# Sagnac/OpticalRayTracing.jl

Measured on NVIDIA B200. Metric: FP64 ray-surface intersections/sec, higher is better.
Workload: dtype f64

## Files before the change

opticalraytracing.jl_b200/csrc/kern_trace3d.cu:

```cuda
#include "kern.cuh"

struct Hit {
    double xs, ys;
    double xf, yf;
    unsigned flags;
    double opl;
};

__device__ __forceinline__ double strict_opl_start(const RayS& r, int mode, double n0, double y, double x, double z0)
{
    if (mode == 1) return SD(SM(n0, -z0), r.k3);
    return SM(n0, SA(SM(x, r.k1), SM(y, r.k2)));
}

__device__ __forceinline__ double strict_opl_close(const RayS& r, const ort_field& f, double nlast)
{
    if (f.opd_radius == 0.0) return r.opl;
    const double qx = SS(r.x, f.opd_xc), qy = SS(r.y, f.opd_yc);
    const double b = SA(SM(qx, r.k1), SM(qy, r.k2));
    const double cq = SS(SA(SM(qx, qx), SM(qy, qy)), SM(f.opd_radius, f.opd_radius));
    const double sg = (f.opd_radius < 0.0) ? -1.0 : 1.0;
    const double tau = SS(-b, SM(sg, SQ(SS(SM(b, b), cq))));
    return SA(r.opl, SM(nlast, tau));
}
// ... 45 lines not shown
    const Hit h = trace_strict_impl<EXT, SurfArray, POLY, true>(S, nsurf, stop, y, x, u, v, fld, n0, nlast, vignette, poly, npoly, &bad);
    if (bad) return trace_strict_cold<EXT, SurfArray, POLY>(S, nsurf, stop, y, x, u, v, fld, n0, nlast, vignette, poly, npoly);
    return h;
}

__device__ __forceinline__ int nonfinite_bit(double a) { return 0x7FEFFFFF - (hi32(a) & 0x7FFFFFFF); }

__device__ __forceinline__ bool is_nan_bits(double a)
{
    return (hi32(a) & 0x7FFFFFFF) > 0x7FF00000 ||
           ((hi32(a) & 0x7FFFFFFF) == 0x7FF00000 && __double2loint(a) != 0);
}

template <int RPT, bool EXT, class SurfArray, bool MIRROR = true, int SIMPLE = 0, bool R2ONLY = false, int POLY = 0, class QT = NoPolyK>
__device__ __forceinline__ void trace_fast(const SurfArray& S, int nsurf, int stop, double n0,
                                           const double* y, const double* x, const double* u,
                                           const double* v, Hit* h, int* amb,
                                           const ort_field* fld = nullptr, double nlast = 1.0, bool vignette = false,
                                           const double* K0 = nullptr, bool kzcheck = true, const double* poly = nullptr,
                                           int npoly = 0, const QT* Q = nullptr)
{
    RaysF<RPT> r;
#pragma unroll
    for (int j = 0; j < RPT; j++) {
        if (K0) {
            r.x[j] = x[j]; r.y[j] = y[j]; r.z[j] = 0.0;
            r.Kx[j] = K0[0]; r.Ky[j] = K0[1]; r.Kz[j] = K0[2];
            r.amb[j] = 0; r.opl[j] = 0.0; r.vig[j] = 0;
        } else fast_init(r, j, n0, y[j], x[j], u[j], v[j]);
        if (EXT) {
            r.opl[j] = (fld->mode == 1) ? fast_div(-(n0 * n0) * fld->z0, r.Kz[j]) : fma(x[j], r.Kx[j], y[j] * r.Ky[j]);
        }
    }
    int i = 0;
    for (; i < stop; i++)
        if constexpr (POLY == 2) fast_step<RPT, EXT, MIRROR, SIMPLE, 2>(S[i], r, vignette, nullptr, 0, 0, &Q->r[i]);
        else fast_step<RPT, EXT, MIRROR, SIMPLE, POLY>(S[i], r, vignette, (POLY && poly) ? poly + (size_t)i * npoly : nullptr, npoly, nsurf * npoly);
#pragma unroll
    for (int j = 0; j < RPT; j++) {
        if (R2ONLY) { h[j].xs = fma(r.x[j], r.x[j], r.y[j] * r.y[j]); h[j].ys = 0.0; }
        else { h[j].xs = r.x[j]; h[j].ys = r.y[j]; }
    }
    for (; i < nsurf; i++)
        if constexpr (POLY == 2) fast_step<RPT, EXT, MIRROR, SIMPLE, 2>(S[i], r, vignette, nullptr, 0, 0, &Q->r[i]);
        else fast_step<RPT, EXT, MIRROR, SIMPLE, POLY>(S[i], r, vignette, (POLY && poly) ? poly + (size_t)i * npoly : nullptr, npoly, nsurf * npoly);
#pragma unroll
    for (int j = 0; j < RPT; j++) {
        h[j].xf = r.x[j]; h[j].yf = r.y[j];
        h[j].flags = (EXT && r.vig[j]) ? ORT_FLAG_VIGN : 0u;
        amb[j] = r.amb[j] | nonfinite_bit(r.x[j]) | nonfinite_bit(r.y[j]);
        if (kzcheck) amb[j] |= nonfinite_bit(r.Kz[j]);
        h[j].opl = 0.0;
        if (EXT) {
            double opl = r.opl[j];
            if (fld->opd_radius != 0.0) {
                const double qx = r.x[j] - fld->opd_xc, qy = r.y[j] - fld->opd_yc;
                const double bK = fma(qx, r.Kx[j], qy * r.Ky[j]);
                const double cq = fma(qx, qx, fma(qy, qy, -fld->opd_radius * fld->opd_radius));
                const double d = fma(bK, bK, -(nlast * nlast) * cq);
                double sq = fast_sqrt(d);
                if ((fld->opd_radius < 0.0) != (nlast < 0.0)) sq = -sq;
                opl = opl - bK - sq;
                amb[j] |= nonfinite_bit(opl);
            }
            h[j].opl = opl;
        }
    }
}

struct RawAcc {
    int n, nflag_lo, nflag_hi;
    double s1x, s2x, s1y, s2y, rmax;
    double s1o, s2o; int nvig;
    int nstrict;
// ... 490 lines not shown
    const unsigned nxu = (unsigned)A.nx;

    for (unsigned tile = blockIdx.x; tile < ntiles; tile += gridDim.x) {
        double y0[RPT], x0[RPT], u[RPT], v[RPT];
        unsigned idx[RPT];
        bool valid[RPT];
#pragma unroll
        for (int j = 0; j < RPT; j++) {
            const unsigned i0 = (tile * RPT + j) * ORT_TILE + threadIdx.x;
            valid[j] = i0 < NN;
            idx[j] = min(i0, NN - 1);
            const unsigned iy = idx[j] / nxu, ix = idx[j] - iy * nxu;
            y0[j] = __ldg(A.ys + (ysoff + iy)); x0[j] = __ldg(A.xs + ix);
            u[j] = 0.0; v[j] = 0.0;
        }
        if (!collimated || ARITH != ORT_ARITH_FAST) {
#pragma unroll
            for (int j = 0; j < RPT; j++) field_slopes(fld, y0[j], x0[j], u[j], v[j]);
        }
        FocusRay q[RPT];
        double xs[RPT], ys[RPT];
        unsigned flg[RPT];
        bool sv[RPT];
        if (ARITH == ORT_ARITH_FAST) {
            RaysF<RPT> r;
#pragma unroll
            for (int j = 0; j < RPT; j++) {
                if (collimated) {
                    r.x[j] = x0[j]; r.y[j] = y0[j]; r.z[j] = 0.0;
                    r.Kx[j] = K0[0]; r.Ky[j] = K0[1]; r.Kz[j] = K0[2];
                    r.amb[j] = 0; r.opl[j] = 0.0; r.vig[j] = 0;
                } else fast_init(r, j, P.n0, y0[j], x0[j], u[j], v[j]);
            }
            const int ns = P.nsurf - 1;
            int i = 0;
            for (; i < A.stop; i++) fast_step<RPT, false, MIRROR, SIMPLE, 0>(P.s[i], r);
#pragma unroll
            for (int j = 0; j < RPT; j++) s_xy[j][threadIdx.x] = make_double2(r.x[j], r.y[j]);
            for (; i < ns; i++) fast_step<RPT, false, MIRROR, SIMPLE, 0>(P.s[i], r);
#pragma unroll
            for (int j = 0; j < RPT; j++) {
                int amb = r.amb[j];
                if (refr_last) {
                    const double Dp = fma(r.Kz[j], r.Kz[j], SL.dn2);
                    amb |= hi32(Dp) - SL.tir_thr;
                    amb |= nonfinite_bit(MIRROR ? sign_of_n2(fast_sqrt(Dp), SL.n2mask) : fast_sqrt(Dp));
                }
                q[j].a0 = r.x[j]; q[j].a1 = r.y[j]; q[j].a2 = r.z[j]; q[j].a3 = r.Kx[j]; q[j].a4 = r.Ky[j];
                q[j].a5 = fast_div_rcp(r.Kz[j]);
                double xa, ya, xb, yb;
                focus_pos_fast(q[j], F.t_lo, xa, ya);
                focus_pos_fast(q[j], F.t_hi, xb, yb);
                amb |= nonfinite_bit(xa) | nonfinite_bit(ya) | nonfinite_bit(xb) | nonfinite_bit(yb);
                const double2 st = s_xy[j][threadIdx.x];
                const double r2 = fma(st.x, st.x, st.y * st.y);
                amb |= tiny_vs_bit(r2 - A.a_stop2, A.a_stop2);
                sv[j] = amb < 0;
                flg[j] = 0u;
            }
        } else {
#pragma unroll
            for (int j = 0; j < RPT; j++) {
                int bad = 0;
                FocusS o = focus_strict_impl<ORT_STRICT_XF>(P, A.stop, y0[j], x0[j], u[j], v[j], &bad);
                if (ORT_STRICT_XF && bad) o = focus_strict_cold(P, A.stop, y0[j], x0[j], u[j], v[j]);
                q[j] = o.q; xs[j] = o.xs; ys[j] = o.ys; flg[j] = o.flags; sv[j] = true;
// ... 435 lines not shown
        double s1x = 0.0, s2x = 0.0, s1y = 0.0, s2y = 0.0, rmax = -CUDART_INF;
        const unsigned edge_b = (unsigned)(A.ny - 1) * nxu;
        if (AIMED && ok && threadIdx.x < 2) {
            double ex, ey, rr; bool keep;
            if (rec[14] == 1.0) { const double* e = rec + 16 + 4 * threadIdx.x; keep = e[0] == 1.0; ex = e[1]; ey = e[2]; rr = e[3]; }
            else {
                const Hit he = trace_strict_cold<false>(s_surf, nsurf, stop, threadIdx.x ? par[1] : par[0], 0.0, par[7], A.v);
                const double ri = jl_hypot(he.xs, he.ys);
                keep = !(ri > par[5] || is_nan_bits(he.xf) || is_nan_bits(he.yf)); ex = he.xf; ey = he.yf - par[8]; rr = ri * ri;
            }
            if (keep) { const double dy = ey - cy; s1x += ex; s2x = fma(ex, ex, s2x); s1y += dy; s2y = fma(dy, dy, s2y); rmax = fmax(rmax, rr); n++; }
        }
        unsigned iyj[CS_RPT], ixj[CS_RPT];
#pragma unroll
        for (int j = 0; j < CS_RPT; j++) { const unsigned i = threadIdx.x + j * CS_THREADS; iyj[j] = i / nxu; ixj[j] = i - iyj[j] * nxu; }
        const double g_y1 = par[0], g_y2 = par[1], g_dy = par[2], g_xe = par[3], g_dx = par[4], a_stop2 = par[6], hpc = par[8] + cy;
        for (unsigned i0 = threadIdx.x; ok && i0 < NN; i0 += step) {
            double y0[CS_RPT], x0[CS_RPT], uu[CS_RPT], vv[CS_RPT];
            bool valid[CS_RPT];
#pragma unroll
            for (int j = 0; j < CS_RPT; j++) {
                const unsigned i = i0 + j * CS_THREADS;
                valid[j] = i < NN && !(AIMED && (i == 0 || i == edge_b));
                const unsigned iy = min(iyj[j], (unsigned)A.ny - 1), ix = ixj[j];
                if (AIMED) {
                    y0[j] = (iy == (unsigned)A.ny - 1) ? g_y2 : SA(g_y1, SM((double)iy, g_dy));
                    x0[j] = (ix == nxu - 1) ? g_xe : SM((double)ix, g_dx);
                } else { y0[j] = __ldg(A.ys + iy); x0[j] = __ldg(A.xs + ix); }
                uu[j] = 0.0; vv[j] = A.v;
                ixj[j] += dr; iyj[j] += dq;
                if (ixj[j] >= nxu) { ixj[j] -= nxu; iyj[j]++; }
            }
            Hit h[CS_RPT]; int amb[CS_RPT];
            trace_fast<CS_RPT, false, SurfK*, false, SIMPLE>(s_surf, nsurf, stop, n0, y0, x0, uu, vv, h, amb, nullptr, 1.0, false, K0);
#pragma unroll
            for (int j = 0; j < CS_RPT; j++) {
                double r2 = fma(h[j].xs, h[j].xs, h[j].ys * h[j].ys);
                amb[j] |= tiny_vs_bit(r2 - a_stop2, a_stop2);
                bool drop = r2 > a_stop2;
                if (amb[j] < 0 && valid[j]) {
                    h[j] = trace_strict_cold<false>(s_surf, nsurf, stop, y0[j], x0[j], par[7], A.v);
                    const double ri = jl_hypot(h[j].xs, h[j].ys);
                    drop = ri > par[5] || is_nan_bits(h[j].xf) || is_nan_bits(h[j].yf);
                    r2 = ri * ri;
                }
                if (valid[j] && !drop) {
                    const double ex = h[j].xf, dy = h[j].yf - hpc;
                    s1x += ex; s2x = fma(ex, ex, s2x); s1y += dy; s2y = fma(dy, dy, s2y);
                    if (r2 > rmax) rmax = r2;
                    n++;
                }
            }
        }
#pragma unroll
        for (int d = 16; d >= 1; d >>= 1) {
            n += __shfl_down_sync(0xffffffffu, n, d);
            s1x += __shfl_down_sync(0xffffffffu, s1x, d); s2x += __shfl_down_sync(0xffffffffu, s2x, d);
            s1y += __shfl_down_sync(0xffffffffu, s1y, d); s2y += __shfl_down_sync(0xffffffffu, s2y, d);
            rmax = fmax(rmax, __shfl_down_sync(0xffffffffu, rmax, d));
        }
        const int lane = threadIdx.x & 31, warp = threadIdx.x >> 5;
        if (lane == 0) { s_redn[warp] = n; s_red[warp][0] = s1x; s_red[warp][1] = s2x; s_red[warp][2] = s1y; s_red[warp][3] = s2y; s_red[warp][4] = rmax; }
        __syncthreads();
        if (threadIdx.x == 0) {
            for (int w = 1; w < CS_THREADS / 32; w++) {
                n += s_redn[w]; s1x += s_red[w][0]; s2x += s_red[w][1]; s1y += s_red[w][2]; s2y += s_red[w][3];
            }
// ... 58 lines not shown
    return arith == ORT_ARITH_FAST ? (variant == 2 ? ORT_SIMPLE_RPT : (variant == 3 ? ORT_SE_RPT : (variant == 4 ? ORT_SC_RPT : ORT_FAST_RPT))) : ORT_STRICT_RPT;
}

int grid_blocks_per_sm(int arith, int variant)
{
    int nb = 0;
    cudaError_t e;
    if (arith == ORT_ARITH_FAST && variant == 2)
        e = cudaOccupancyMaxActiveBlocksPerMultiprocessor(&nb, k_grid<ORT_ARITH_FAST, ORT_SIMPLE_RPT, 0, 1, false, true>, ORT_TILE, 0);
    else if (arith == ORT_ARITH_FAST && variant == 3)
        e = cudaOccupancyMaxActiveBlocksPerMultiprocessor(&nb, k_grid<ORT_ARITH_FAST, ORT_SE_RPT, 2, 0, false, true>, ORT_TILE, 0);
    else if (arith == ORT_ARITH_FAST && variant == 4)
        e = cudaOccupancyMaxActiveBlocksPerMultiprocessor(&nb, k_grid<ORT_ARITH_FAST, ORT_SC_RPT, 0, 1, false, 2>, ORT_TILE, 0);
    else if (arith == ORT_ARITH_FAST)
        e = variant ? cudaOccupancyMaxActiveBlocksPerMultiprocessor(&nb, k_grid<ORT_ARITH_FAST, ORT_FAST_RPT, 1>, ORT_TILE, 0)
                    : cudaOccupancyMaxActiveBlocksPerMultiprocessor(&nb, k_grid<ORT_ARITH_FAST, ORT_FAST_RPT, 0>, ORT_TILE, 0);
    else
        e = (variant & 1) ? cudaOccupancyMaxActiveBlocksPerMultiprocessor(&nb, k_grid<ORT_ARITH_STRICT, ORT_STRICT_RPT, 1>, ORT_TILE, 0)
                          : cudaOccupancyMaxActiveBlocksPerMultiprocessor(&nb, k_grid<ORT_ARITH_STRICT, ORT_STRICT_RPT, 0>, ORT_TILE, 0);
    if (e != cudaSuccess || nb < 1) nb = 1;
    return nb;
}

cudaError_t launch_grid(const Presc& P, const GridArgs& A, int arith, dim3 grid, cudaStream_t st, const PolyK* Q)
{
    const bool ext = A.ext != 0 || P.poly != nullptr;
    if (arith == ORT_ARITH_FAST) {
        const bool others = A.r || A.theta || A.wx || A.wy || A.flags || A.opd;
        const bool lean = !ext && !others && A.ex && A.ey && A.mask;
        const bool stats_only = !ext && !others && !A.ex && !A.ey && !A.mask;
        const int variant = grid_variant(P, arith, ext);
        const bool simple = variant == 2;
        const bool lean_opd = (A.ext & ORT_EXT_OPD) && A.ex && A.ey && A.mask && A.opd && !(A.r || A.theta || A.wx || A.wy || A.flags);
        if (variant == 3 && !(A.ext & ORT_EXT_VIGNETTE) && lean_opd) k_grid<ORT_ARITH_FAST, ORT_SE_RPT, 2, 1, false, true><<<grid, ORT_TILE, 0, st>>>(P, A, NoPolyK());
        else if (variant == 3 && !(A.ext & ORT_EXT_VIGNETTE)) k_grid<ORT_ARITH_FAST, ORT_SE_RPT, 2, 0, false, true><<<grid, ORT_TILE, 0, st>>>(P, A, NoPolyK());
        else if (variant == 3 && lean_opd) k_grid<ORT_ARITH_FAST, ORT_SE_RPT, 1, 1, false, true><<<grid, ORT_TILE, 0, st>>>(P, A, NoPolyK());
        else if (variant == 3) k_grid<ORT_ARITH_FAST, ORT_SE_RPT, 1, 0, false, true><<<grid, ORT_TILE, 0, st>>>(P, A, NoPolyK());
        else if (variant == 4 && lean) k_grid<ORT_ARITH_FAST, ORT_SC_RPT, 0, 1, false, 2><<<grid, ORT_TILE, 0, st>>>(P, A, NoPolyK());
        else if (variant == 4 && stats_only) k_grid<ORT_ARITH_FAST, ORT_SC_RPT, 0, 2, false, 2><<<grid, ORT_TILE, 0, st>>>(P, A, NoPolyK());
        else if (variant == 4) k_grid<ORT_ARITH_FAST, ORT_SC_RPT, 0, 0, false, 2><<<grid, ORT_TILE, 0, st>>>(P, A, NoPolyK());
        else if (simple && lean) k_grid<ORT_ARITH_FAST, ORT_SIMPLE_RPT, 0, 1, false, true><<<grid, ORT_TILE, 0, st>>>(P, A, NoPolyK());
        else if (simple && stats_only) k_grid<ORT_ARITH_FAST, ORT_SIMPLE_RPT, 0, 2, false, true><<<grid, ORT_TILE, 0, st>>>(P, A, NoPolyK());
        else if (simple) k_grid<ORT_ARITH_FAST, ORT_SIMPLE_RPT, 0, 0, false, true><<<grid, ORT_TILE, 0, st>>>(P, A, NoPolyK());
        else if (P.poly && Q && !A.ext && !others && A.ex && A.ey && A.mask) k_grid<ORT_ARITH_FAST, ORT_FAST_RPT, 0, 1, false, 0, 2><<<grid, ORT_TILE, 0, st>>>(P, A, *Q);
        else if (P.poly && Q) k_grid<ORT_ARITH_FAST, ORT_FAST_RPT, 1, 0, false, 0, 2><<<grid, ORT_TILE, 0, st>>>(P, A, *Q);
        else if (P.poly && !A.ext && !others && A.ex && A.ey && A.mask) k_grid<ORT_ARITH_FAST, ORT_FAST_RPT, 0, 1, false, 0, 1><<<grid, ORT_TILE, 0, st>>>(P, A, NoPolyK());
        else if (P.poly) k_grid<ORT_ARITH_FAST, ORT_FAST_RPT, 1, 0, false, 0, 1><<<grid, ORT_TILE, 0, st>>>(P, A, NoPolyK());
        else if (ext && !P.has_mirror) k_grid<ORT_ARITH_FAST, ORT_FAST_RPT, 1, 0, false><<<grid, ORT_TILE, 0, st>>>(P, A, NoPolyK());
        else if (ext) k_grid<ORT_ARITH_FAST, ORT_FAST_RPT, 1><<<grid, ORT_TILE, 0, st>>>(P, A, NoPolyK());
        else if (lean && !P.has_mirror) k_grid<ORT_ARITH_FAST, ORT_FAST_RPT, 0, 1, false><<<grid, ORT_TILE, 0, st>>>(P, A, NoPolyK());
        else if (stats_only && !P.has_mirror) k_grid<ORT_ARITH_FAST, ORT_FAST_RPT, 0, 2, false><<<grid, ORT_TILE, 0, st>>>(P, A, NoPolyK());
        else if (!P.has_mirror) k_grid<ORT_ARITH_FAST, ORT_FAST_RPT, 0, 0, false><<<grid, ORT_TILE, 0, st>>>(P, A, NoPolyK());
        else if (lean) k_grid<ORT_ARITH_FAST, ORT_FAST_RPT, 0, 1><<<grid, ORT_TILE, 0, st>>>(P, A, NoPolyK());
        else if (stats_only) k_grid<ORT_ARITH_FAST, ORT_FAST_RPT, 0, 2><<<grid, ORT_TILE, 0, st>>>(P, A, NoPolyK());
        else k_grid<ORT_ARITH_FAST, ORT_FAST_RPT, 0><<<grid, ORT_TILE, 0, st>>>(P, A, NoPolyK());
    } else {
        if (ext) k_grid<ORT_ARITH_STRICT, ORT_STRICT_RPT, 1><<<grid, ORT_TILE, 0, st>>>(P, A, NoPolyK());
        else k_grid<ORT_ARITH_STRICT, ORT_STRICT_RPT, 0><<<grid, ORT_TILE, 0, st>>>(P, A, NoPolyK());
    }
    return cudaGetLastError();
}

cudaError_t launch_grid_finalize(const RawPart* partials, int nparts, int n_fields, ort_stats* stats,
                                 cudaStream_t st)
{
    k_grid_finalize<<<n_fields, 256, 0, st>>>(partials, nparts, stats);
    return cudaGetLastError();
}

size_t compact_tile_ints(unsigned NN)
{
    const size_t ntiles = (NN + ORT_TILE - 1) / ORT_TILE;
    return ntiles + ntiles / SCAN_CHUNK + 2;
}

static cudaError_t launch_tile_scan(int* tile_counts, unsigned ntiles, int n_fields, cudaStream_t st)
{
    const unsigned nchunks = (ntiles + SCAN_CHUNK - 1) / SCAN_CHUNK;
    k_tile_scan<<<dim3(nchunks, n_fields), 256, 0, st>>>(tile_counts, tile_counts + (size_t)n_fields * ntiles, ntiles, nchunks);
    k_chunk_scan<<<n_fields, 256, 0, st>>>(tile_counts + (size_t)n_fields * ntiles, nchunks);
    return cudaGetLastError();
}

cudaError_t launch_compact(int* tile_counts, const CompactArgs& C, int n_fields, cudaStream_t st)
{
    const unsigned ntiles = (C.NN + ORT_TILE - 1) / ORT_TILE;
    cudaError_t e = launch_tile_scan(tile_counts, ntiles, n_fields, st);
    if (e != cudaSuccess) return e;
    k_compact<<<dim3(ntiles, n_fields), ORT_TILE, 0, st>>>(C);
    return cudaGetLastError();
}

int focus_blocks_per_sm(int arith, int variant)
{
    int nb = 0;
    cudaError_t e;
    if (arith != ORT_ARITH_FAST) e = cudaOccupancyMaxActiveBlocksPerMultiprocessor(&nb, k_focus<ORT_ARITH_STRICT, ORT_STRICT_RPT, true, 0>, ORT_TILE, 0);
    else if (variant == 2) e = cudaOccupancyMaxActiveBlocksPerMultiprocessor(&nb, k_focus<ORT_ARITH_FAST, ORT_SIMPLE_RPT, false, 1>, ORT_TILE, 0);
    else if (variant == 4) e = cudaOccupancyMaxActiveBlocksPerMultiprocessor(&nb, k_focus<ORT_ARITH_FAST, ORT_SC_RPT, false, 2>, ORT_TILE, 0);
    else e = cudaOccupancyMaxActiveBlocksPerMultiprocessor(&nb, k_focus<ORT_ARITH_FAST, ORT_FAST_RPT, true, 0>, ORT_TILE, 0);
    if (e != cudaSuccess || nb < 1) nb = 1;
    return nb;
}

cudaError_t launch_focus(const Presc& P, const FocusArgs& F, int arith, dim3 grid, cudaStream_t st)
{
    if (arith == ORT_ARITH_FAST) {
        const int variant = grid_variant(P, arith, 0);
        if (variant == 2) k_focus<ORT_ARITH_FAST, ORT_SIMPLE_RPT, false, 1><<<grid, ORT_TILE, 0, st>>>(P, F);
        else if (variant == 4) k_focus<ORT_ARITH_FAST, ORT_SC_RPT, false, 2><<<grid, ORT_TILE, 0, st>>>(P, F);
        else if (!P.has_mirror) k_focus<ORT_ARITH_FAST, ORT_FAST_RPT, false, 0><<<grid, ORT_TILE, 0, st>>>(P, F);
        else k_focus<ORT_ARITH_FAST, ORT_FAST_RPT, true, 0><<<grid, ORT_TILE, 0, st>>>(P, F);
    } else {
        k_focus<ORT_ARITH_STRICT, ORT_STRICT_RPT, true, 0><<<grid, ORT_TILE, 0, st>>>(P, F);
    }
    return cudaGetLastError();
}

cudaError_t launch_compact_focus(int* tile_counts, const CompactArgs& C, int n_fields, int n_foci, cudaStream_t st)
{
    const unsigned ntiles = (C.NN + ORT_TILE - 1) / ORT_TILE;
    cudaError_t e = launch_tile_scan(tile_counts, ntiles, n_fields, st);
    if (e != cudaSuccess) return e;
    k_compact_focus<<<dim3(ntiles, n_fields), ORT_TILE, 0, st>>>(C, n_foci);
    return cudaGetLastError();
}

cudaError_t launch_rays(const Presc& P, const RaysArgs& A, int arith, cudaStream_t st)
{
    const unsigned nb = (unsigned)((A.N + 255) / 256);
    if (nb == 0) return cudaSuccess;
    const bool ext = A.opl != nullptr || P.has_apertures || P.poly != nullptr;
    if (arith == ORT_ARITH_FAST) {
        if (ext) k_rays<ORT_ARITH_FAST, true><<<nb, 256, 0, st>>>(P, A);
        else k_rays<ORT_ARITH_FAST, false><<<nb, 256, 0, st>>>(P, A);
    } else {
        if (ext) k_rays<ORT_ARITH_STRICT, true><<<nb, 256, 0, st>>>(P, A);
        else k_rays<ORT_ARITH_STRICT, false><<<nb, 256, 0, st>>>(P, A);
    }
    return cudaGetLastError();
}

// ... 42 lines not shown
```

opticalraytracing.jl_b200/csrc/ort_api.cu:

```cuda
#include <math.h>
#include <stdarg.h>
#include <stddef.h>
#include <stdio.h>
#include <string.h>

#include <new>
#include <vector>

#ifndef _GNU_SOURCE
#define _GNU_SOURCE
#endif
#include <sched.h>
#include <stdlib.h>
#include <sys/syscall.h>
#include <unistd.h>
#include "ort_ctx.cuh"

thread_local char g_init_err[512] = "";

int ort_fail(ort_ctx* c, int code, const char* fmt, ...)
{
    va_list ap;
    va_start(ap, fmt);
    vsnprintf(c ? c->err : g_init_err, 512, fmt, ap);
// ... 183 lines not shown
    void* p = nullptr;
    if (cudaHostAlloc(&p, bytes ? bytes : 8, cudaHostAllocDefault) != cudaSuccess) return nullptr;
    return p;
}
void ort_host_free(void* p) { if (p) cudaFreeHost(p); }

int64_t ort_launch_count(ort_ctx* ctx) { return ctx ? ctx->launches : 0; }

int ort_profile_enable(ort_ctx* ctx, int on)
{
    if (!ctx) return ORT_EINVAL;
    ctx->prof_on = on ? 1 : 0;
    ctx->prof_n = 0;
    return ORT_OK;
}

int ort_profile_read(ort_ctx* ctx, double* ms_out, int max_n)
{
    if (!ctx || !ms_out || max_n < 0) return ORT_EINVAL;
    long long n = ctx->prof_n < 64 ? ctx->prof_n : 64;
    if (n > max_n) n = max_n;
    const long long first = ctx->prof_n - n;
    for (long long j = 0; j < n; j++) {
        const int slot = (int)((first + j) % 64);
        if (cudaEventSynchronize(ctx->prof_ev[slot][1]) != cudaSuccess) return ORT_ECUDA;
        float t = 0.f;
        if (cudaEventElapsedTime(&t, ctx->prof_ev[slot][0], ctx->prof_ev[slot][1]) != cudaSuccess) return ORT_ECUDA;
        ms_out[j] = (double)t;
    }
    ctx->prof_n = 0;
    return (int)n;
}

int ort_set_layout(ort_ctx* ctx, int rows, const double* R, const double* t, const double* n, const double* K)
{
    if (!ctx) return ORT_EINVAL;
    if (!R || !t || !n) return fail(ctx, ORT_EINVAL, "ort_set_layout: NULL column");
    if (rows < 2 || rows > ORT_MAX_ROWS) return fail(ctx, ORT_EINVAL, "ort_set_layout: rows = %d not in [2, %d]", rows, ORT_MAX_ROWS);
    Presc& P = ctx->presc;
    memset(&P, 0, sizeof P);
    P.nsurf = rows - 1;
    P.fast_ok = 1;
    P.t_last = t[rows - 1];
    P.n0 = n[0];
    P.nlast = n[rows - 1];
    for (int i = 0; i + 1 < rows; i++) {
        const double Ri = R[i + 1], Ki = K ? K[i + 1] : 0.0;
        derive_surface(P.s[i], Ri, Ki, t[i], n[i], n[i + 1]);
        if (Ri == 0.0 || isnan(Ri) || !isfinite(Ki) || !isfinite(t[i]) || !isfinite(n[i]) || !isfinite(n[i + 1]) ||
            n[i] == 0.0 || n[i + 1] == 0.0)
            P.fast_ok = 0;
        if (!(n[i] > 0.0) || !(n[i + 1] > 0.0)) P.has_mirror = 1;
    }
    const double L = gap_scale(t, rows);
    P.simple = P.fast_ok && !P.has_mirror;
    bool conic_class = P.simple, any_conic = false;
    for (int i = 0; i + 1 < rows; i++) {
        const bool plane = (P.s[i].kcode & SURF_KIND_MASK) == SURF_PLANE;
        if (!plane && !(P.s[i].kcode & SURF_REFR)) conic_class = false;
        if ((P.s[i].kcode & SURF_KIND_MASK) == SURF_CONIC) any_conic = true;
        if (!simple_surface(P.s[i], L)) P.simple = 0;
    }
    if (!P.simple && conic_class && any_conic) P.simple = 2;
    ctx->rows = rows;
    ctx->have_layout = true;
    ctx->fast_ok_layout = P.fast_ok;
    return ORT_OK;
}

int ort_set_polynomials(ort_ctx* ctx, int rows, int ncoef, const double* coef)
{
    if (!ctx) return ORT_EINVAL;
    if (!ctx->have_layout) return fail(ctx, ORT_EINVAL, "ort_set_polynomials: call ort_set_layout first");
    Presc& P = ctx->presc;
    auto clear = [&]() {
        P.poly = nullptr; P.npoly = 0; P.fast_ok = ctx->fast_ok_layout; ctx->have_polyk = false;
        for (int i = 0; i < P.nsurf; i++) P.s[i].kcode = P.s[i].kind & 7;
    };
    if (!coef || ncoef <= 0) { clear(); return ORT_OK; }
    if (rows != ctx->rows) return fail(ctx, ORT_EINVAL, "ort_set_polynomials: rows = %d, layout has %d", rows, ctx->rows);
    if (ncoef > ORT_MAX_POLY) return fail(ctx, ORT_EINVAL, "ort_set_polynomials: ncoef = %d > %d", ncoef, ORT_MAX_POLY);
    bool any = false;
    for (int i = 0; i < rows * ncoef; i++) {
        if (isnan(coef[i])) return fail(ctx, ORT_EINVAL, "ort_set_polynomials: NaN coefficient");
        any = any || coef[i] != 0.0;
    }
    if (!any) { clear(); return ORT_OK; }
    CK(cudaSetDevice(ctx->device));
    ScratchScope scratch(ctx, ctx->stream);
    const size_t ntab = (size_t)(rows - 1) * ncoef;
    double* d_c; ENSURE(SL_POLY, 2 * ntab * 8, d_c);
    std::vector<double> tab(2 * ntab);
    for (size_t i = 0; i < ntab; i++) { tab[i] = coef[ncoef + i]; tab[ntab + i] = (double)(i % ncoef) * coef[ncoef + i]; }
    CK(cudaMemcpyAsync(d_c, tab.data(), 2 * ntab * 8, cudaMemcpyHostToDevice, ctx->stream));
    CK(cudaStreamSynchronize(ctx->stream));
    P.poly = d_c; P.npoly = ncoef;
// ... 991 lines not shown
```

opticalraytracing.jl_b200/csrc/ort_internal.cuh:

```cuda
#pragma once
#include <cuda_runtime.h>
#include <math_constants.h>
#include <stdint.h>

#include "ort_b200.h"

#define ORT_TILE 256

enum { SURF_PLANE = 0, SURF_SPHERE = 1, SURF_CONIC = 2, SURF_KIND_MASK = 3, SURF_REFR = 4, SURF_N2NEG = (int)0x80000000 };
enum { SURF_KCODE_POLY = 7 };

struct SurfK {
    double R, K, t, n1, n2, sgnR;
    double c;
    double cn1sq;
    double n1sq;
    double dn2;
    double onepK;
    int32_t kind;
    int32_t tir_thr;
    int32_t gr_thr;
    int32_t n2mask;
    int32_t eq_thr;
    int32_t kcode;
    double a, a2;
    double Rsq;
    double eta, etasq;
    double inv_cn1sq;
    double c2n1sq, m2cn1sq;
};
#define ORT_INF (__builtin_huge_val())
#ifndef ORT_GUARD_BAND
#define ORT_GUARD_BAND 2.44140625e-4
#endif
#if defined(__CUDACC__)
#define ORT_HD __host__ __device__
#else
#define ORT_HD
#endif
ORT_HD inline int32_t ort_hi_word(double a)
{
#if defined(__CUDA_ARCH__)
    return __double2hiint(a);
#else
    int64_t b; memcpy(&b, &a, 8); return (int32_t)(b >> 32);
#endif
}
ORT_HD inline void derive_surface(SurfK& S, double R, double K, double t, double n1, double n2)
{
    const bool finiteR = (R - R) == 0.0;
    S.R = R; S.K = K; S.t = t; S.n1 = n1; S.n2 = n2;
    S.sgnR = (R < 0.0) ? -1.0 : ((R > 0.0) ? 1.0 : R);
    S.c = finiteR ? 1.0 / R : 0.0;
    S.n1sq = n1 * n1;
    S.cn1sq = S.c * S.n1sq;
    S.dn2 = (n2 - n1) * (n2 + n1);
    S.onepK = 1.0 + K;
    S.kind = (!finiteR ? SURF_PLANE : (K == 0.0 ? SURF_SPHERE : SURF_CONIC)) | (n1 != n2 ? SURF_REFR : 0) |
             (n2 < 0.0 ? SURF_N2NEG : 0);
    S.kcode = S.kind & 7;
    S.tir_thr = ort_hi_word(n2 * n2 * ORT_GUARD_BAND);
    S.gr_thr = ort_hi_word(n1 * n1 * ORT_GUARD_BAND);
    S.n2mask = (n2 < 0.0) ? (int32_t)0x80000000 : 0;
    const int32_t e = finiteR ? ort_hi_word(fabs(R) * (1.0 - 9.5367431640625e-07)) : 0x7FF00000;
    S.eq_thr = (R < 0.0) ? (int32_t)(0x80000000u + (uint32_t)(e - 1)) : e - 1;
    S.a = ORT_INF; S.a2 = ORT_INF;
    S.inv_cn1sq = 0.0; S.c2n1sq = 0.0; S.m2cn1sq = 0.0;
    S.Rsq = R * R; S.eta = n1 / n2; S.etasq = S.eta * S.eta;
}

#define ORT_NODIV_MAX_R_OVER_L 64.0
ORT_HD inline bool simple_surface(SurfK& S, double L)
{
    if (S.kcode == SURF_PLANE || S.kcode == (SURF_PLANE | SURF_REFR)) return S.n1 > 0.0 && S.n2 > 0.0;
    if (S.kcode != (SURF_SPHERE | SURF_REFR) || !(S.n1 > 0.0) || !(S.n2 > 0.0)) return false;
    if (!(fabs(S.R) <= ORT_NODIV_MAX_R_OVER_L * L) || S.cn1sq == 0.0 || (S.cn1sq - S.cn1sq) != 0.0) return false;
    S.inv_cn1sq = 1.0 / S.cn1sq;
    S.c2n1sq = S.cn1sq * S.c; S.m2cn1sq = -2.0 * S.cn1sq;
    return true;
}
ORT_HD inline double gap_scale(const double* t, int n)
{
    double L = 0.0;
    for (int i = 0; i < n; i++) { const double a = fabs(t[i]); if ((a - a) == 0.0) L += a; }
    return L;
}

struct Presc {
    int32_t nsurf;
    int32_t fast_ok;
    int32_t has_apertures;
    int32_t has_mirror;
    const double* poly;
    int32_t npoly;
    int32_t simple;
    double n0;
    double nlast;
    double t_last;
    SurfK s[ORT_MAX_ROWS - 1];
};

#define ORT_POLYK_N 10
struct PolyRow { double c[ORT_POLYK_N], d[ORT_POLYK_N]; };
struct PolyK { PolyRow r[ORT_MAX_ROWS - 1]; };
struct NoPolyK {};
template <int POLYK> struct PolyArg { typedef NoPolyK type; };
template <> struct PolyArg<2> { typedef PolyK type; };

struct Part {
    long long n;
    double mx, my, m2x, m2y, rmax;
    int nmiss, ntir, ndom, nclip;
};

__device__ __forceinline__ void part_zero(Part& p)
{
    p.n = 0; p.mx = p.my = p.m2x = p.m2y = 0.0; p.rmax = -CUDART_INF;
    p.nmiss = p.ntir = p.ndom = p.nclip = 0;
}

__device__ __forceinline__ void part_merge(Part& a, const Part& b)
{
    a.nmiss += b.nmiss; a.ntir += b.ntir; a.ndom += b.ndom; a.nclip += b.nclip;
    if (b.n == 0) return;
    if (a.n == 0) { a.n = b.n; a.mx = b.mx; a.my = b.my; a.m2x = b.m2x; a.m2y = b.m2y; a.rmax = b.rmax; return; }
    double na = (double)a.n, nb = (double)b.n, n = na + nb;
    double w = nb / n;
    double dx = b.mx - a.mx, dy = b.my - a.my;
// ... 265 lines not shown
    return fma(r, e, r);
}

#define EXP_BAND (30 << 20)
__device__ __forceinline__ bool nonneg_finite(double a) { return (unsigned)hi32(a) < 0x7FF00000u; }
__device__ __forceinline__ int tiny_vs_bit(double a, double b)
{
    return ((hi32(a) & 0x7FFFFFFF) + EXP_BAND) - (hi32(b) & 0x7FFFFFFF);
}
__device__ __forceinline__ bool tiny_vs(double a, double b) { return tiny_vs_bit(a, b) < 0; }
__device__ __forceinline__ int equator_bit(double mz)
{
    const int h = hi32(mz);
    return (~h) | (int)((unsigned)h - 0xBEB00001u);
}

template <int RPT>
struct RaysF {
    double x[RPT], y[RPT], z[RPT], Kx[RPT], Ky[RPT], Kz[RPT];
    int amb[RPT];
    double opl[RPT];
    int vig[RPT];
};

template <int RPT>
__device__ __forceinline__ void fast_init(RaysF<RPT>& r, int j, double n0, double y, double x, double u, double v)
{
    const double inv = n0 * fast_rsqrt(fma(v, v, fma(u, u, 1.0)));
    r.x[j] = x; r.y[j] = y; r.z[j] = 0.0;
    r.Kx[j] = v * inv; r.Ky[j] = u * inv; r.Kz[j] = inv;
    r.amb[j] = 0; r.opl[j] = 0.0; r.vig[j] = 0;
}

template <int RPT>
__device__ __forceinline__ void fast_ext(const SurfK& S, RaysF<RPT>& r, int j, double s, bool vignette)
{
    r.opl[j] = fma(S.n1sq, s, r.opl[j]);
    if (vignette) {
        const double r2 = fma(r.x[j], r.x[j], r.y[j] * r.y[j]);
        r.amb[j] |= tiny_vs_bit(r2 - S.a2, S.a2);
        r.vig[j] |= (r2 > S.a2) ? 1 : 0;
    }
}

template <int RPT, bool EXT = false, bool MIRROR = true, int SIMPLE = 0, int POLY = 0>
__device__ __forceinline__ void fast_step(const SurfK& S, RaysF<RPT>& r, bool vignette = false, const double* pc = nullptr,
                                          int npoly = 0, int dstride = 0, const PolyRow* q = nullptr)
{
    const int kc = S.kcode;
    const double t = S.t;
    const double c = S.c;
    const double neg1 = -1.0;
    const int gthr = S.gr_thr;
    if (SIMPLE == 1 && kc == (SURF_SPHERE | SURF_REFR)) {
        const double inv = S.inv_cn1sq, c2n1sq = S.c2n1sq, m2cn1sq = S.m2cn1sq;
        const int eqt = S.eq_thr;
        {
            const double dn2 = S.dn2;
            const int thr = S.tir_thr, n2m = S.n2mask;
#pragma unroll
            for (int j = 0; j < RPT; j++) {
                const double zr = r.z[j] - t;
                const double PD = fma(r.x[j], r.Kx[j], fma(r.y[j], r.Ky[j], zr * r.Kz[j]));
                const double P2 = fma(r.x[j], r.x[j], fma(r.y[j], r.y[j], zr * zr));
                const double G = fma(-c, PD, r.Kz[j]);
                const double cF = fma(c2n1sq, P2, m2cn1sq * zr);
                const double disc = fma(G, G, -cF);
                const double ssq = (MIRROR ? copysign(fast_sqrt(disc), r.Kz[j]) : fast_sqrt(disc));
                const double s = (G - ssq) * inv;
                r.x[j] = fma(s, r.Kx[j], r.x[j]);
                r.y[j] = fma(s, r.Ky[j], r.y[j]);
                r.z[j] = fma(s, r.Kz[j], zr);
                if (EXT) fast_ext<RPT>(S, r, j, s, vignette);
                const double Dp = disc + dn2;
                r.amb[j] |= (hi32(disc) - gthr) | (MIRROR ? (hi32(G) ^ hi32(r.Kz[j])) : (hi32(G) | hi32(r.Kz[j]))) | (eqt - hi32(r.z[j])) | (hi32(Dp) - thr);
                const double g = ssq - (MIRROR ? sign_of_n2(fast_sqrt(Dp), n2m) : fast_sqrt(Dp));
                const double gc = g * c;
                r.Kx[j] = fma(gc, r.x[j], r.Kx[j]);
                r.Ky[j] = fma(gc, r.y[j], r.Ky[j]);
                r.Kz[j] = fma(gc, r.z[j], r.Kz[j] - g);
            }
        }
        return;
    }
    if (SIMPLE == 0 && kc == (SURF_SPHERE | SURF_REFR)) {
        const double cn1sq = S.cn1sq;
        const int eqt = S.eq_thr;
        {
            const double dn2 = S.dn2;
            const int thr = S.tir_thr, n2m = S.n2mask;
#pragma unroll
            for (int j = 0; j < RPT; j++) {
                const double zr = r.z[j] - t;
                const double PD = fma(r.x[j], r.Kx[j], fma(r.y[j], r.Ky[j], zr * r.Kz[j]));
                const double P2 = fma(r.x[j], r.x[j], fma(r.y[j], r.y[j], zr * zr));
                const double F = fma(c, P2, -2.0 * zr);
                const double G = fma(-c, PD, r.Kz[j]);
                const double cF = cn1sq * F;
                const double disc = fma(G, G, -cF);
                const double ssq = (MIRROR ? copysign(fast_sqrt(disc), r.Kz[j]) : fast_sqrt(disc));
                const double s = fast_div(F, G + ssq);
                r.x[j] = fma(s, r.Kx[j], r.x[j]);
                r.y[j] = fma(s, r.Ky[j], r.y[j]);
                r.z[j] = fma(s, r.Kz[j], zr);
                if (EXT) fast_ext<RPT>(S, r, j, s, vignette);
                const double Dp = disc + dn2;
                r.amb[j] |= (hi32(disc) - gthr) | (MIRROR ? (hi32(G) ^ hi32(r.Kz[j])) : (hi32(G) | hi32(r.Kz[j]))) | (eqt - hi32(r.z[j])) | (hi32(Dp) - thr);
                const double g = ssq - (MIRROR ? sign_of_n2(fast_sqrt(Dp), n2m) : fast_sqrt(Dp));
                const double gc = g * c;
                r.Kx[j] = fma(gc, r.x[j], r.Kx[j]);
                r.Ky[j] = fma(gc, r.y[j], r.Ky[j]);
                r.Kz[j] = fma(gc, r.z[j], r.Kz[j] - g);
            }
        }
        return;
    }
    if (kc == (SURF_PLANE | SURF_REFR)) {
        {
            const double dn2 = S.dn2;
            const int thr = S.tir_thr, n2m = S.n2mask;
#pragma unroll
            for (int j = 0; j < RPT; j++) {
                const double s = fast_div(t - r.z[j], r.Kz[j]);
                r.x[j] = fma(s, r.Kx[j], r.x[j]);
                r.y[j] = fma(s, r.Ky[j], r.y[j]);
                r.z[j] = 0.0;
                if (EXT) fast_ext<RPT>(S, r, j, s, vignette);
                const double Dp = fma(r.Kz[j], r.Kz[j], dn2);
                r.amb[j] |= hi32(Dp) - thr;
                r.Kz[j] = (MIRROR ? sign_of_n2(fast_sqrt(Dp), n2m) : fast_sqrt(Dp));
            }
        }
        return;
    }
    if (SIMPLE == 1 || kc == SURF_PLANE) {
        {
#pragma unroll
            for (int j = 0; j < RPT; j++) {
                const double s = fast_div(t - r.z[j], r.Kz[j]);
                r.x[j] = fma(s, r.Kx[j], r.x[j]);
                r.y[j] = fma(s, r.Ky[j], r.y[j]);
                r.z[j] = 0.0;
                if (EXT) fast_ext<RPT>(S, r, j, s, vignette);
            }
        }
        return;
    }
    if (SIMPLE == 0 && kc == SURF_SPHERE) {
        const double cn1sq = S.cn1sq;
        const int eqt = S.eq_thr;
        {
#pragma unroll
            for (int j = 0; j < RPT; j++) {
                const double zr = r.z[j] - t;
                const double PD = fma(r.x[j], r.Kx[j], fma(r.y[j], r.Ky[j], zr * r.Kz[j]));
                const double P2 = fma(r.x[j], r.x[j], fma(r.y[j], r.y[j], zr * zr));
                const double F = fma(c, P2, -2.0 * zr);
                const double G = fma(-c, PD, r.Kz[j]);
                const double cF = cn1sq * F;
                const double disc = fma(G, G, -cF);
                const double ssq = (MIRROR ? copysign(fast_sqrt(disc), r.Kz[j]) : fast_sqrt(disc));
                const double s = fast_div(F, G + ssq);
                r.x[j] = fma(s, r.Kx[j], r.x[j]);
                r.y[j] = fma(s, r.Ky[j], r.y[j]);
                r.z[j] = fma(s, r.Kz[j], zr);
                if (EXT) fast_ext<RPT>(S, r, j, s, vignette);
                r.amb[j] |= (hi32(disc) - gthr) | (MIRROR ? (hi32(G) ^ hi32(r.Kz[j])) : (hi32(G) | hi32(r.Kz[j]))) | (eqt - hi32(r.z[j]));
            }
        }
        return;
    }
    if (POLY && kc == SURF_KCODE_POLY) {
        const double onepK = S.onepK, Kc = S.K, n1sq = S.n1sq, dn2 = S.dn2, Rsq = S.Rsq, sgn = S.sgnR;
        const int thr = S.tir_thr;
        const bool refr = (S.kind & SURF_REFR) != 0;
#pragma unroll
        for (int j = 0; j < RPT; j++) {
            const double zr = r.z[j] - t;
// ... 18 lines not shown
            r.x[j] = fma(s, r.Kx[j], r.x[j]);
            r.y[j] = fma(s, r.Ky[j], r.y[j]);
            r.z[j] = fma(s, r.Kz[j], zr);
            if (EXT) fast_ext<RPT>(S, r, j, s, vignette);
            const double r2 = fma(r.x[j], r.x[j], r.y[j] * r.y[j]);
            const double Dt = fma(-r2, onepK, Rsq);
            r.amb[j] |= (hi32(disc) - gthr) | hi32(G) | hi32(r.Kz[j]) | hi32(Dt) | ((hi32(Dt) + (20 << 20)) - hi32(Rsq));
            const double rs = sgn * fast_rsqrt(Dt);
            double dpx = 0.0, dpy = 0.0;
            if (POLY == 2) {
                dpx = dpy = q->d[ORT_POLYK_N - 1];
#pragma unroll
                for (int k = ORT_POLYK_N - 2; k >= 1; k--) { dpx = fma(dpx, r.x[j], q->d[k]); dpy = fma(dpy, r.y[j], q->d[k]); }
            } else {
                for (int k = npoly - 1; k >= 1; k--) {
                    const double ck = __ldg(pc + dstride + k);
                    dpx = fma(dpx, r.x[j], ck); dpy = fma(dpy, r.y[j], ck);
                }
            }
            const double m1 = fma(r.x[j], rs, dpx), m2 = fma(r.y[j], rs, dpy);
            if (refr) {
                const double q = fma(m1, m1, fma(m2, m2, 1.0));
                const double b = r.Kz[j] - fma(r.Kx[j], m1, r.Ky[j] * m2);
                const double Dq = fma(b, b, dn2 * q);
                r.amb[j] |= ((hi32(Dq) - (hi32(q) - 0x3FF00000)) - thr) | hi32(b);
                const double g = fast_div(b - fast_sqrt(Dq), q);
                r.Kx[j] = fma(g, m1, r.Kx[j]);
                r.Ky[j] = fma(g, m2, r.Ky[j]);
                r.Kz[j] = r.Kz[j] - g;
            }
        }
        return;
    }
    if (SIMPLE != 1) {
        const double onepK = S.onepK, Kc = S.K, n1sq = S.n1sq, dn2 = S.dn2;
        const int thr = S.tir_thr, n2m = S.n2mask;
        const bool refr = SIMPLE == 2 || (kc & SURF_REFR) != 0;
#pragma unroll
        for (int j = 0; j < RPT; j++) {
            const double zr = r.z[j] - t;
            const double zk = onepK * zr;
            const double PD = fma(r.x[j], r.Kx[j], fma(r.y[j], r.Ky[j], zk * r.Kz[j]));
            const double P2 = fma(r.x[j], r.x[j], fma(r.y[j], r.y[j], zk * zr));
            const double F = fma(c, P2, -2.0 * zr);
            const double G = fma(-c, PD, r.Kz[j]);
            const double cAF = c * F * fma(Kc, r.Kz[j] * r.Kz[j], n1sq);
            const double disc = fma(G, G, -cAF);
            const double ssq = (MIRROR ? copysign(fast_sqrt(disc), r.Kz[j]) : fast_sqrt(disc));
            const double s = fast_div(F, G + ssq);
            r.x[j] = fma(s, r.Kx[j], r.x[j]);
            r.y[j] = fma(s, r.Ky[j], r.y[j]);
            r.z[j] = fma(s, r.Kz[j], zr);
            if (EXT) fast_ext<RPT>(S, r, j, s, vignette);
            const double mz = fma(c * onepK, r.z[j], neg1);
            r.amb[j] |= (hi32(disc) - gthr) | (MIRROR ? (hi32(G) ^ hi32(r.Kz[j])) : (hi32(G) | hi32(r.Kz[j]))) | equator_bit(mz);
            if (refr) {
                const double cx = c * r.x[j], cy = c * r.y[j];
                const double q = fma(cx, cx, fma(cy, cy, mz * mz));
                const double Dq = fma(dn2, q, disc);
                r.amb[j] |= (hi32(Dq) - (hi32(q) - 0x3FF00000)) - thr;
                const double g = fast_div(ssq - (MIRROR ? sign_of_n2(fast_sqrt(Dq), n2m) : fast_sqrt(Dq)), q);
                r.Kx[j] = fma(g, cx, r.Kx[j]);
                r.Ky[j] = fma(g, cy, r.Ky[j]);
                r.Kz[j] = fma(g, mz, r.Kz[j]);
            }
        }
    }
// ... 2 lines not shown
```

Measured before the change: 404.5 billion.

## Fold sphere discriminant constants to drop P2 computation in simple refractive path

Adds an algebraic fold for all-spherical refractive systems. The squared radial distance is carried in the z slot, so each sphere step computes the discriminant from precomputed per-surface constants (fold_A, fold_B) instead of rebuilding P2 from x, y and zr. This saves a few FMAs per ray-surface step. Precomputation happens at layout time, gated by an environment variable and a radius-ratio accuracy check, with the old path kept as template variant 3. It relies on a bitmask trick on z and may change rounding behaviour.

```diff
diff --git a/opticalraytracing.jl_b200/csrc/kern_trace3d.cu b/opticalraytracing.jl_b200/csrc/kern_trace3d.cu
--- a/opticalraytracing.jl_b200/csrc/kern_trace3d.cu
+++ b/opticalraytracing.jl_b200/csrc/kern_trace3d.cu
@@ -101,14 +101,20 @@
             r.opl[j] = (fld->mode == 1) ? fast_div(-(n0 * n0) * fld->z0, r.Kz[j]) : fma(x[j], r.Kx[j], y[j] * r.Ky[j]);
         }
     }
+    fold_start<SIMPLE>(S[0], r);
     int i = 0;
     for (; i < stop; i++)
         if constexpr (POLY == 2) fast_step<RPT, EXT, MIRROR, SIMPLE, 2>(S[i], r, vignette, nullptr, 0, 0, &Q->r[i]);
         else fast_step<RPT, EXT, MIRROR, SIMPLE, POLY>(S[i], r, vignette, (POLY && poly) ? poly + (size_t)i * npoly : nullptr, npoly, nsurf * npoly);
-#pragma unroll
-    for (int j = 0; j < RPT; j++) {
-        if (R2ONLY) { h[j].xs = fma(r.x[j], r.x[j], r.y[j] * r.y[j]); h[j].ys = 0.0; }
-        else { h[j].xs = r.x[j]; h[j].ys = r.y[j]; }
+    if (SIMPLE == 1 && R2ONLY && stop > 0 && S[stop - 1].fold_w) {
+#pragma unroll
+        for (int j = 0; j < RPT; j++) { h[j].xs = r.z[j]; h[j].ys = 0.0; }
+    } else {
+#pragma unroll
+        for (int j = 0; j < RPT; j++) {
+            if (R2ONLY) { h[j].xs = fma(r.x[j], r.x[j], r.y[j] * r.y[j]); h[j].ys = 0.0; }
+            else { h[j].xs = r.x[j]; h[j].ys = r.y[j]; }
+        }
     }
     for (; i < nsurf; i++)
         if constexpr (POLY == 2) fast_step<RPT, EXT, MIRROR, SIMPLE, 2>(S[i], r, vignette, nullptr, 0, 0, &Q->r[i]);
@@ -665,6 +671,7 @@
                     r.amb[j] = 0; r.opl[j] = 0.0; r.vig[j] = 0;
                 } else fast_init(r, j, P.n0, y0[j], x0[j], u[j], v[j]);
             }
+            fold_start<SIMPLE>(P.s[0], r);
             const int ns = P.nsurf - 1;
             int i = 0;
             for (; i < A.stop; i++) fast_step<RPT, false, MIRROR, SIMPLE, 0>(P.s[i], r);
@@ -1166,7 +1173,7 @@
                 if (ixj[j] >= nxu) { ixj[j] -= nxu; iyj[j]++; }
             }
             Hit h[CS_RPT]; int amb[CS_RPT];
-            trace_fast<CS_RPT, false, SurfK*, false, SIMPLE>(s_surf, nsurf, stop, n0, y0, x0, uu, vv, h, amb, nullptr, 1.0, false, K0);
+            trace_fast<CS_RPT, false, SurfK*, false, SIMPLE == 1 ? 3 : SIMPLE>(s_surf, nsurf, stop, n0, y0, x0, uu, vv, h, amb, nullptr, 1.0, false, K0);
 #pragma unroll
             for (int j = 0; j < CS_RPT; j++) {
                 double r2 = fma(h[j].xs, h[j].xs, h[j].ys * h[j].ys);
@@ -1291,16 +1298,29 @@
         const int variant = grid_variant(P, arith, ext);
         const bool simple = variant == 2;
         const bool lean_opd = (A.ext & ORT_EXT_OPD) && A.ex && A.ey && A.mask && A.opd && !(A.r || A.theta || A.wx || A.wy || A.flags);
-        if (variant == 3 && !(A.ext & ORT_EXT_VIGNETTE) && lean_opd) k_grid<ORT_ARITH_FAST, ORT_SE_RPT, 2, 1, false, true><<<grid, ORT_TILE, 0, st>>>(P, A, NoPolyK());
-        else if (variant == 3 && !(A.ext & ORT_EXT_VIGNETTE)) k_grid<ORT_ARITH_FAST, ORT_SE_RPT, 2, 0, false, true><<<grid, ORT_TILE, 0, st>>>(P, A, NoPolyK());
-        else if (variant == 3 && lean_opd) k_grid<ORT_ARITH_FAST, ORT_SE_RPT, 1, 1, false, true><<<grid, ORT_TILE, 0, st>>>(P, A, NoPolyK());
-        else if (variant == 3) k_grid<ORT_ARITH_FAST, ORT_SE_RPT, 1, 0, false, true><<<grid, ORT_TILE, 0, st>>>(P, A, NoPolyK());
+        const bool fold = P.fold != 0;
+        if (variant == 3 && !(A.ext & ORT_EXT_VIGNETTE) && lean_opd) {
+            if (fold) k_grid<ORT_ARITH_FAST, ORT_SE_RPT, 2, 1, false, 1><<<grid, ORT_TILE, 0, st>>>(P, A, NoPolyK());
+            else k_grid<ORT_ARITH_FAST, ORT_SE_RPT, 2, 1, false, 3><<<grid, ORT_TILE, 0, st>>>(P, A, NoPolyK());
+        } else if (variant == 3 && !(A.ext & ORT_EXT_VIGNETTE)) {
+            if (fold) k_grid<ORT_ARITH_FAST, ORT_SE_RPT, 2, 0, false, 1><<<grid, ORT_TILE, 0, st>>>(P, A, NoPolyK());
+            else k_grid<ORT_ARITH_FAST, ORT_SE_RPT, 2, 0, false, 3><<<grid, ORT_TILE, 0, st>>>(P, A, NoPolyK());
+        } else if (variant == 3 && lean_opd) {
+            if (fold) k_grid<ORT_ARITH_FAST, ORT_SE_RPT, 1, 1, false, 1><<<grid, ORT_TILE, 0, st>>>(P, A, NoPolyK());
+            else k_grid<ORT_ARITH_FAST, ORT_SE_RPT, 1, 1, false, 3><<<grid, ORT_TILE, 0, st>>>(P, A, NoPolyK());
+        } else if (variant == 3) {
+            if (fold) k_grid<ORT_ARITH_FAST, ORT_SE_RPT, 1, 0, false, 1><<<grid, ORT_TILE, 0, st>>>(P, A, NoPolyK());
+            else k_grid<ORT_ARITH_FAST, ORT_SE_RPT, 1, 0, false, 3><<<grid, ORT_TILE, 0, st>>>(P, A, NoPolyK());
+        }
         else if (variant == 4 && lean) k_grid<ORT_ARITH_FAST, ORT_SC_RPT, 0, 1, false, 2><<<grid, ORT_TILE, 0, st>>>(P, A, NoPolyK());
         else if (variant == 4 && stats_only) k_grid<ORT_ARITH_FAST, ORT_SC_RPT, 0, 2, false, 2><<<grid, ORT_TILE, 0, st>>>(P, A, NoPolyK());
         else if (variant == 4) k_grid<ORT_ARITH_FAST, ORT_SC_RPT, 0, 0, false, 2><<<grid, ORT_TILE, 0, st>>>(P, A, NoPolyK());
-        else if (simple && lean) k_grid<ORT_ARITH_FAST, ORT_SIMPLE_RPT, 0, 1, false, true><<<grid, ORT_TILE, 0, st>>>(P, A, NoPolyK());
-        else if (simple && stats_only) k_grid<ORT_ARITH_FAST, ORT_SIMPLE_RPT, 0, 2, false, true><<<grid, ORT_TILE, 0, st>>>(P, A, NoPolyK());
-        else if (simple) k_grid<ORT_ARITH_FAST, ORT_SIMPLE_RPT, 0, 0, false, true><<<grid, ORT_TILE, 0, st>>>(P, A, NoPolyK());
+        else if (simple && lean && fold) k_grid<ORT_ARITH_FAST, ORT_SIMPLE_RPT, 0, 1, false, 1><<<grid, ORT_TILE, 0, st>>>(P, A, NoPolyK());
+        else if (simple && lean) k_grid<ORT_ARITH_FAST, ORT_SIMPLE_RPT, 0, 1, false, 3><<<grid, ORT_TILE, 0, st>>>(P, A, NoPolyK());
+        else if (simple && stats_only && fold) k_grid<ORT_ARITH_FAST, ORT_SIMPLE_RPT, 0, 2, false, 1><<<grid, ORT_TILE, 0, st>>>(P, A, NoPolyK());
+        else if (simple && stats_only) k_grid<ORT_ARITH_FAST, ORT_SIMPLE_RPT, 0, 2, false, 3><<<grid, ORT_TILE, 0, st>>>(P, A, NoPolyK());
+        else if (simple && fold) k_grid<ORT_ARITH_FAST, ORT_SIMPLE_RPT, 0, 0, false, 1><<<grid, ORT_TILE, 0, st>>>(P, A, NoPolyK());
+        else if (simple) k_grid<ORT_ARITH_FAST, ORT_SIMPLE_RPT, 0, 0, false, 3><<<grid, ORT_TILE, 0, st>>>(P, A, NoPolyK());
         else if (P.poly && Q && !A.ext && !others && A.ex && A.ey && A.mask) k_grid<ORT_ARITH_FAST, ORT_FAST_RPT, 0, 1, false, 0, 2><<<grid, ORT_TILE, 0, st>>>(P, A, *Q);
         else if (P.poly && Q) k_grid<ORT_ARITH_FAST, ORT_FAST_RPT, 1, 0, false, 0, 2><<<grid, ORT_TILE, 0, st>>>(P, A, *Q);
         else if (P.poly && !A.ext && !others && A.ex && A.ey && A.mask) k_grid<ORT_ARITH_FAST, ORT_FAST_RPT, 0, 1, false, 0, 1><<<grid, ORT_TILE, 0, st>>>(P, A, NoPolyK());
@@ -1366,7 +1386,8 @@
 {
     if (arith == ORT_ARITH_FAST) {
         const int variant = grid_variant(P, arith, 0);
-        if (variant == 2) k_focus<ORT_ARITH_FAST, ORT_SIMPLE_RPT, false, 1><<<grid, ORT_TILE, 0, st>>>(P, F);
+        if (variant == 2 && P.fold) k_focus<ORT_ARITH_FAST, ORT_SIMPLE_RPT, false, 1><<<grid, ORT_TILE, 0, st>>>(P, F);
+        else if (variant == 2) k_focus<ORT_ARITH_FAST, ORT_SIMPLE_RPT, false, 3><<<grid, ORT_TILE, 0, st>>>(P, F);
         else if (variant == 4) k_focus<ORT_ARITH_FAST, ORT_SC_RPT, false, 2><<<grid, ORT_TILE, 0, st>>>(P, F);
         else if (!P.has_mirror) k_focus<ORT_ARITH_FAST, ORT_FAST_RPT, false, 0><<<grid, ORT_TILE, 0, st>>>(P, F);
         else k_focus<ORT_ARITH_FAST, ORT_FAST_RPT, true, 0><<<grid, ORT_TILE, 0, st>>>(P, F);
diff --git a/opticalraytracing.jl_b200/csrc/ort_api.cu b/opticalraytracing.jl_b200/csrc/ort_api.cu
--- a/opticalraytracing.jl_b200/csrc/ort_api.cu
+++ b/opticalraytracing.jl_b200/csrc/ort_api.cu
@@ -239,6 +239,12 @@
     return (int)n;
 }
 
+static bool ort_simple_fold()
+{
+    static const bool fold = [] { const char* e = getenv("ORT_SIMPLE_FOLD"); return !e || atoi(e) != 0; }();
+    return fold;
+}
+
 int ort_set_layout(ort_ctx* ctx, int rows, const double* R, const double* t, const double* n, const double* K)
 {
     if (!ctx) return ORT_EINVAL;
@@ -269,6 +275,7 @@
         if (!simple_surface(P.s[i], L)) P.simple = 0;
     }
     if (!P.simple && conic_class && any_conic) P.simple = 2;
+    P.fold = P.simple == 1 && fold_constants(P.s, P.nsurf, L) && ort_simple_fold();
     ctx->rows = rows;
     ctx->have_layout = true;
     ctx->fast_ok_layout = P.fast_ok;
diff --git a/opticalraytracing.jl_b200/csrc/ort_internal.cuh b/opticalraytracing.jl_b200/csrc/ort_internal.cuh
--- a/opticalraytracing.jl_b200/csrc/ort_internal.cuh
+++ b/opticalraytracing.jl_b200/csrc/ort_internal.cuh
@@ -28,6 +28,9 @@
     double eta, etasq;
     double inv_cn1sq;
     double c2n1sq, m2cn1sq;
+    double fold_A, fold_B;
+    int32_t fold_m;
+    int32_t fold_w;
 };
 #define ORT_INF (__builtin_huge_val())
 #ifndef ORT_GUARD_BAND
@@ -66,6 +69,7 @@
     S.eq_thr = (R < 0.0) ? (int32_t)(0x80000000u + (uint32_t)(e - 1)) : e - 1;
     S.a = ORT_INF; S.a2 = ORT_INF;
     S.inv_cn1sq = 0.0; S.c2n1sq = 0.0; S.m2cn1sq = 0.0;
+    S.fold_A = 0.0; S.fold_B = 0.0; S.fold_m = 0; S.fold_w = 0;
     S.Rsq = R * R; S.eta = n1 / n2; S.etasq = S.eta * S.eta;
 }
 
@@ -84,6 +88,30 @@
     double L = 0.0;
     for (int i = 0; i < n; i++) { const double a = fabs(t[i]); if ((a - a) == 0.0) L += a; }
     return L;
+}
+
+#define ORT_FOLD_MAX_PAIR_OVER_L 64.0
+ORT_HD inline bool fold_constants(SurfK* s, int n, double L)
+{
+    const int sph = SURF_SPHERE | SURF_REFR;
+    bool ok = true;
+    for (int i = 0; i < n; i++) {
+        SurfK& S = s[i];
+        S.fold_w = (S.kcode != sph && i + 1 < n && s[i + 1].kcode == sph) ? 1 : 0;
+        if (S.kcode != sph) continue;
+        const double t = S.t;
+        S.fold_B = t * fma(S.c2n1sq, t, -S.m2cn1sq);
+        if (i > 0 && s[i - 1].kcode == sph) {
+            const double Rp = s[i - 1].R;
+            if (!(Rp * Rp <= ORT_FOLD_MAX_PAIR_OVER_L * L * fabs(S.R))) ok = false;
+            S.fold_m = -1;
+            S.fold_A = fma(2.0 * S.c2n1sq, Rp - t, S.m2cn1sq);
+        } else {
+            S.fold_m = 0;
+            S.fold_A = S.c2n1sq;
+        }
+    }
+    return ok;
 }
 
 struct Presc {
@@ -94,6 +122,7 @@
     const double* poly;
     int32_t npoly;
     int32_t simple;
+    int32_t fold;
     double n0;
     double nlast;
     double t_last;
@@ -425,6 +454,24 @@
     r.amb[j] = 0; r.opl[j] = 0.0; r.vig[j] = 0;
 }
 
+template <int SIMPLE, int RPT>
+__device__ __forceinline__ void fold_start(const SurfK& S0, RaysF<RPT>& r)
+{
+    if (SIMPLE == 1 && S0.kcode == (SURF_SPHERE | SURF_REFR)) {
+#pragma unroll
+        for (int j = 0; j < RPT; j++) r.z[j] = fma(r.x[j], r.x[j], r.y[j] * r.y[j]);
+    }
+}
+
+template <int SIMPLE, int RPT>
+__device__ __forceinline__ void fold_after_plane(const SurfK& S, RaysF<RPT>& r)
+{
+    if (SIMPLE == 1 && S.fold_w) {
+#pragma unroll
+        for (int j = 0; j < RPT; j++) r.z[j] = fma(r.x[j], r.x[j], r.y[j] * r.y[j]);
+    }
+}
+
 template <int RPT>
 __device__ __forceinline__ void fast_ext(const SurfK& S, RaysF<RPT>& r, int j, double s, bool vignette)
 {
@@ -440,25 +487,37 @@
 __device__ __forceinline__ void fast_step(const SurfK& S, RaysF<RPT>& r, bool vignette = false, const double* pc = nullptr,
                                           int npoly = 0, int dstride = 0, const PolyRow* q = nullptr)
 {
+    constexpr bool NODIV = SIMPLE == 1 || SIMPLE == 3;
     const int kc = S.kcode;
     const double t = S.t;
     const double c = S.c;
     const double neg1 = -1.0;
     const int gthr = S.gr_thr;
-    if (SIMPLE == 1 && kc == (SURF_SPHERE | SURF_REFR)) {
+    if (NODIV && kc == (SURF_SPHERE | SURF_REFR)) {
         const double inv = S.inv_cn1sq, c2n1sq = S.c2n1sq, m2cn1sq = S.m2cn1sq;
+        const double fA = S.fold_A, fB = S.fold_B;
+        const int fm = S.fold_m;
         const int eqt = S.eq_thr;
         {
             const double dn2 = S.dn2;
             const int thr = S.tir_thr, n2m = S.n2mask;
 #pragma unroll
             for (int j = 0; j < RPT; j++) {
-                const double zr = r.z[j] - t;
+                double zr, disc;
+                if (SIMPLE == 1) {
+                    zr = __hiloint2double(__double2hiint(r.z[j]) & fm, __double2loint(r.z[j]) & fm) - t;
+                } else {
+                    zr = r.z[j] - t;
+                }
                 const double PD = fma(r.x[j], r.Kx[j], fma(r.y[j], r.Ky[j], zr * r.Kz[j]));
-                const double P2 = fma(r.x[j], r.x[j], fma(r.y[j], r.y[j], zr * zr));
                 const double G = fma(-c, PD, r.Kz[j]);
-                const double cF = fma(c2n1sq, P2, m2cn1sq * zr);
-                const double disc = fma(G, G, -cF);
+                if (SIMPLE == 1) {
+                    disc = fma(-fA, r.z[j], fma(G, G, -fB));
+                } else {
+                    const double P2 = fma(r.x[j], r.x[j], fma(r.y[j], r.y[j], zr * zr));
+                    const double cF = fma(c2n1sq, P2, m2cn1sq * zr);
+                    disc = fma(G, G, -cF);
+                }
                 const double ssq = (MIRROR ? copysign(fast_sqrt(disc), r.Kz[j]) : fast_sqrt(disc));
                 const double s = (G - ssq) * inv;
                 r.x[j] = fma(s, r.Kx[j], r.x[j]);
@@ -524,9 +583,10 @@
                 r.Kz[j] = (MIRROR ? sign_of_n2(fast_sqrt(Dp), n2m) : fast_sqrt(Dp));
             }
         }
+        fold_after_plane<SIMPLE>(S, r);
         return;
     }
-    if (SIMPLE == 1 || kc == SURF_PLANE) {
+    if (NODIV || kc == SURF_PLANE) {
         {
 #pragma unroll
             for (int j = 0; j < RPT; j++) {
@@ -537,6 +597,7 @@
                 if (EXT) fast_ext<RPT>(S, r, j, s, vignette);
             }
         }
+        fold_after_plane<SIMPLE>(S, r);
         return;
     }
     if (SIMPLE == 0 && kc == SURF_SPHERE) {
@@ -621,7 +682,7 @@
         }
         return;
     }
-    if (SIMPLE != 1) {
+    if (!NODIV) {
         const double onepK = S.onepK, Kc = S.K, n1sq = S.n1sq, dn2 = S.dn2;
         const int thr = S.tir_thr, n2m = S.n2mask;
         const bool refr = SIMPLE == 2 || (kc & SURF_REFR) != 0;
```

Result: no change. 408.0 billion, median of 6 (+0.9%).
